# gylien/scale-letkf

Measured on AMD Instinct MI355X. Metric: grid-point LETKF solves/sec, higher is better.
Workload: dtype f64

## Files before the change

### scale-letkf_amd/csrc/letkf_search.hip

```cpp

#include <hip/hip_runtime.h>
#include <limits.h>
#include <stdint.h>
#include <stdio.h>

#include "../../include/letkf_amd.h"
#include "letkf_device.h"
#include "letkf_divby_dev.h"
#include "letkf_lane_dev.h"
#include "letkf_search_dev.h"

namespace letkf {

namespace {

using namespace search_dev;

__device__ __forceinline__ unsigned long long key_bits(int criterion, const CalOut& c) {
  if (criterion == 1) return (unsigned long long)__double_as_longlong(c.ndist);
  if (criterion == 2) return 0x7FFFFFFFFFFFFFFFull - (unsigned long long)__double_as_longlong(c.rloc);
  return (unsigned long long)__double_as_longlong(c.rdiag);
}

enum Pass { kCount = 0, kEmitAll = 1, kHist = 2, kEmitSelect = 3 };

}

struct SelState {
  unsigned long long prefix;
  int shift;
  unsigned long long thresh;
  int tie_budget;
  int emitted;
};

template <int PASS>
__device__ __forceinline__ int sweep_group(const SearchArgs& A, const int gs, const int ge, const double ri,
                                           const double rj, const double rlev, const double rz, const long out,
                                           SelState& st, unsigned int* hist) {
  const letkf_search_tables& t = A.t;
  const int lane = threadIdx.x & 63;
  const unsigned long long lt_mask = (lane == 0) ? 0ull : (~0ull >> (64 - lane));
  int cnt = 0;
  for (int m = gs; m < ge; ++m) {
    const int ic = t.group_member[m];
    const double dzi = t.hori_loc[ic] * kDistZeroFac / t.dx;
    const double dzj = t.hori_loc[ic] * kDistZeroFac / t.dy;
    int imin, imax, jmin, jmax;
    ij_obsgrd_ext(t, ic, ri - dzi, rj - dzj, imin, jmin);
    ij_obsgrd_ext(t, ic, ri + dzi, rj + dzj, imax, jmax);
    imin = max(imin, 1);
    jmin = max(jmin, 1);
    imax = min(imax, t.ngrdext_i[ic]);
    jmax = min(jmax, t.ngrdext_j[ic]);
    if (imin > imax || jmin > jmax) continue;
    const long acb = t.ac_off[ic];
    const int ld = t.ngrdext_i[ic] + 1;
    for (int j = jmin; j <= jmax; ++j) {
      const int lo = t.ac_ext[acb + (imin - 1) + (long)ld * (j - 1)];
      const int hi = t.ac_ext[acb + imax + (long)ld * (j - 1)];
      for (int base = lo; base < hi; base += 64) {
        const int row = base + lane;
        CalOut c{0.0, -1.0, -1.0};
        if (row < hi) c = local_cal(t, ic, ri, rj, rlev, rz, row);
        bool acc = c.rloc != 0.0;
        unsigned long long key = 0;
        if (PASS >= kHist && acc) key = key_bits(t.criterion, c);
        if (PASS == kHist) {
          if (acc && (st.shift == 56 || (key >> (st.shift + 8)) == st.prefix))
            atomicAdd(&hist[(unsigned int)(key >> st.shift) & 0xFFu], 1u);
          continue;
        }
        bool tie = false;
        if (PASS == kEmitSelect) {
          tie = acc && key == st.thresh;
          acc = acc && key < st.thresh;
        }
        const unsigned long long mk = __ballot(acc);
        const int pos = __popcll(mk & lt_mask);
        if (PASS != kCount && acc) {
          const long o = out + st.emitted + pos;
          A.obs_idx[o] = row;
          A.rdiag_l[o] = c.rdiag;
          A.rloc_l[o] = c.rloc;
        }
        const int na = __popcll(mk);
        cnt += na;
        if (PASS != kCount) st.emitted += na;
        if (PASS == kEmitSelect) {
          const unsigned long long tk = __ballot(tie);
          const int tpos = __popcll(tk & lt_mask);
          if (tie && tpos < st.tie_budget) {
            const long o = out + st.emitted + tpos;
            A.obs_idx[o] = row;
            A.rdiag_l[o] = c.rdiag;
            A.rloc_l[o] = c.rloc;
          }
          const int nt = min(__popcll(tk), st.tie_budget);
          st.tie_budget -= nt;
          st.emitted += nt;
          cnt += nt;
        }
      }
    }
  }
  return cnt;
}

__device__ __forceinline__ int wave_incl_scan(int v) {
  v += __builtin_amdgcn_update_dpp(0, v, 0x111, 0xF, 0xF, false);
  v += __builtin_amdgcn_update_dpp(0, v, 0x112, 0xF, 0xF, false);
  v += __builtin_amdgcn_update_dpp(0, v, 0x114, 0xF, 0xF, false);
  v += __builtin_amdgcn_update_dpp(0, v, 0x118, 0xF, 0xF, false);
  v += __builtin_amdgcn_update_dpp(0, v, 0x142, 0xA, 0xF, false);
  v += __builtin_amdgcn_update_dpp(0, v, 0x143, 0xC, 0xF, false);
  return v;
}

__device__ __forceinline__ void find_bin(const unsigned int* hist, const int want, int& bsel, int& before) {
  const int lane = threadIdx.x & 63;
  const uint4 h = *reinterpret_cast<const uint4*>(&hist[4 * lane]);
  const int s = (int)(h.x + h.y + h.z + h.w);
  const int incl = wave_incl_scan(s);
  const int excl = incl - s;
  const bool here = excl < want && incl >= want;
  int b = 4 * lane, cum = excl;
  if (cum + (int)h.x < want) {
    cum += (int)h.x;
    ++b;
    if (cum + (int)h.y < want) {
      cum += (int)h.y;
      ++b;
      if (cum + (int)h.z < want) {
        cum += (int)h.z;
        ++b;
      }
    }
  }
  const unsigned long long mk = __ballot(here);
  if (mk == 0ull) {
    bsel = 255;
    before = __builtin_amdgcn_readlane(incl, 63) - __builtin_amdgcn_readfirstlane((int)hist[255]);
    return;
  }
  const int src = __ffsll((long long)mk) - 1;
  bsel = __builtin_amdgcn_readlane(b, src);
  before = __builtin_amdgcn_readlane(cum, src);
}

constexpr int kCacheCap = 512;

__device__ __forceinline__ int cache_group(const SearchArgs& A, const int gs, const int ge, const double ri,
                                           const double rj, const double rlev, const double rz, double* cache) {
  const letkf_search_tables& t = A.t;
  const int lane = threadIdx.x & 63;
  const unsigned long long lt_mask = (lane == 0) ? 0ull : (~0ull >> (64 - lane));
  int cnt = 0;
  for (int m = gs; m < ge; ++m) {
    const int ic = t.group_member[m];
    const double dzi = t.hori_loc[ic] * kDistZeroFac / t.dx;
    const double dzj = t.hori_loc[ic] * kDistZeroFac / t.dy;
    int imin, imax, jmin, jmax;
    ij_obsgrd_ext(t, ic, ri - dzi, rj - dzj, imin, jmin);
    ij_obsgrd_ext(t, ic, ri + dzi, rj + dzj, imax, jmax);
    imin = max(imin, 1);
    jmin = max(jmin, 1);
    imax = min(imax, t.ngrdext_i[ic]);
    jmax = min(jmax, t.ngrdext_j[ic]);
    if (imin > imax || jmin > jmax) continue;
    const long acb = t.ac_off[ic];
    const int ld = t.ngrdext_i[ic] + 1;
    for (int j = jmin; j <= jmax; ++j) {
      const int lo = t.ac_ext[acb + (imin - 1) + (long)ld * (j - 1)];
      const int hi = t.ac_ext[acb + imax + (long)ld * (j - 1)];
      for (int base = lo; base < hi; base += 64) {
        const int row = base + lane;
        CalOut c{0.0, -1.0, -1.0};
        if (row < hi) c = local_cal(t, ic, ri, rj, rlev, rz, row);
        const bool acc = c.rloc != 0.0;
        const unsigned long long mk = __ballot(acc);
        const int na = __popcll(mk);
        if (cnt + na > kCacheCap) return -1;
        if (acc) {
          const int e = cnt + __popcll(mk & lt_mask);
          *reinterpret_cast<double2*>(&cache[4 * e]) =
              double2{__longlong_as_double((long long)key_bits(t.criterion, c)), __longlong_as_double((long long)row)};
          *reinterpret_cast<double2*>(&cache[4 * e + 2]) = double2{c.rdiag, c.rloc};
        }
        cnt += na;
      }
    }
  }
  return cnt;
}

__device__ __forceinline__ int select_from_cache(const SearchArgs& A, const int nc, const int nmax, const long out,
                                                 const double* cache, unsigned int* hist) {
  const int lane = threadIdx.x & 63;
  const unsigned long long lt_mask = (lane == 0) ? 0ull : (~0ull >> (64 - lane));
  __builtin_amdgcn_fence(__ATOMIC_RELEASE, "wavefront");
  __builtin_amdgcn_wave_barrier();
  __builtin_amdgcn_fence(__ATOMIC_ACQUIRE, "wavefront");
  unsigned long long thresh = ~0ull;
  int tie_budget = 0;
  if (nc > nmax) {
    unsigned long long prefix = 0ull;
    int want = nmax;
    for (int round = 0; round < 8; ++round) {
      for (int b = lane; b < 256; b += 64) hist[b] = 0;
      __builtin_amdgcn_fence(__ATOMIC_RELEASE, "wavefront");
      __builtin_amdgcn_wave_barrier();
      const int shift = 56 - 8 * round;
      for (int e = lane; e < nc; e += 64) {
        const unsigned long long key = (unsigned long long)__double_as_longlong(cache[4 * e]);
        if (round == 0 || (key >> (shift + 8)) == prefix) atomicAdd(&hist[(unsigned int)(key >> shift) & 0xFFu], 1u);
      }
      __builtin_amdgcn_fence(__ATOMIC_ACQ_REL, "wavefront");
      __builtin_amdgcn_wave_barrier();
      int cum = 0, bsel = 255;
      find_bin(hist, want, bsel, cum);
      want -= cum;
      prefix = (round == 0) ? (unsigned long long)bsel : ((prefix << 8) | (unsigned long long)bsel);
    }
    thresh = prefix;
    tie_budget = want;
  }
  int emitted = 0;
  for (int e0 = 0; e0 < nc; e0 += 64) {
    const int e = e0 + lane;
    bool acc = false, tie = false;
    double2 a2{0.0, 0.0}, b2{0.0, 0.0};
    if (e < nc) {
      a2 = *reinterpret_cast<const double2*>(&cache[4 * e]);
      b2 = *reinterpret_cast<const double2*>(&cache[4 * e + 2]);
      const unsigned long long key = (unsigned long long)__double_as_longlong(a2.x);
      acc = nc <= nmax || key < thresh;
      tie = nc > nmax && key == thresh;
    }
    const unsigned long long mk = __ballot(acc);
    if (acc) {
      const long o = out + emitted + __popcll(mk & lt_mask);
      A.obs_idx[o] = (int)__double_as_longlong(a2.y);
      A.rdiag_l[o] = b2.x;
      A.rloc_l[o] = b2.y;
    }
    emitted += __popcll(mk);
    const unsigned long long tk = __ballot(tie);
    const int tpos = __popcll(tk & lt_mask);
    if (tie && tpos < tie_budget) {
      const long o = out + emitted + tpos;
      A.obs_idx[o] = (int)__double_as_longlong(a2.y);
      A.rdiag_l[o] = b2.x;
      A.rloc_l[o] = b2.y;
    }
    const int nt = min(__popcll(tk), tie_budget);
    tie_budget -= nt;
    emitted += nt;
  }
  return emitted;
}

__global__ void __launch_bounds__(256) letkf_search_kernel(const SearchArgs A) {
  __shared__ unsigned int hist_all[4][256];
  extern __shared__ __attribute__((aligned(16))) double cache_all[];
  const letkf_search_tables& t = A.t;
  const int lane = threadIdx.x & 63;
  const int wv = __builtin_amdgcn_readfirstlane(threadIdx.x >> 6);
  unsigned int* hist = hist_all[wv];
  double* cache = cache_all + (size_t)wv * 4 * kCacheCap;

  for (long pt = (long)blockIdx.x * 4 + wv; pt < A.npts; pt += (long)gridDim.x * 4) {
    const double ri = A.ri[pt], rj = A.rj[pt], rlev = A.rlev[pt], rz = A.rz[pt];
    long out = A.fill ? A.obs_off[pt] : 0;
    int total = 0;

    for (int ig = 0; ig < t.ngroup; ++ig) {
      const int gs = t.group_start[ig], ge = t.group_start[ig + 1];
      const int nmax = t.max_nobs[t.group_member[gs]];
      SelState st{0ull, 56, 0ull, 0, 0};
      int ngrp = 0;
      if (nmax <= 0) {
        ngrp = A.fill ? sweep_group<kEmitAll>(A, gs, ge, ri, rj, rlev, rz, out, st, hist)
                      : sweep_group<kCount>(A, gs, ge, ri, rj, rlev, rz, out, st, hist);
      } else if (A.fill && (ngrp = cache_group(A, gs, ge, ri, rj, rlev, rz, cache)) >= 0) {
        ngrp = select_from_cache(A, ngrp, nmax, out, cache, hist);
        __builtin_amdgcn_fence(__ATOMIC_RELEASE, "wavefront");
        __builtin_amdgcn_wave_barrier();
      } else {
        const int cnt = sweep_group<kCount>(A, gs, ge, ri, rj, rlev, rz, out, st, hist);
        if (cnt <= nmax) {
          ngrp = cnt;
          if (A.fill) sweep_group<kEmitAll>(A, gs, ge, ri, rj, rlev, rz, out, st, hist);
        } else if (!A.fill) {
          ngrp = nmax;
        } else {
          int want = nmax;
          for (int round = 0; round < 8; ++round) {
            for (int b = lane; b < 256; b += 64) hist[b] = 0;
            __builtin_amdgcn_fence(__ATOMIC_RELEASE, "wavefront");
            __builtin_amdgcn_wave_barrier();
            st.shift = 56 - 8 * round;
            sweep_group<kHist>(A, gs, ge, ri, rj, rlev, rz, out, st, hist);
            __builtin_amdgcn_fence(__ATOMIC_ACQ_REL, "wavefront");
            __builtin_amdgcn_wave_barrier();
            int cum = 0, bsel = 255;
            find_bin(hist, want, bsel, cum);
            want -= cum;
            st.prefix = (round == 0) ? (unsigned long long)bsel : ((st.prefix << 8) | (unsigned long long)bsel);
          }
          st.thresh = st.prefix;
          st.tie_budget = want;
          st.emitted = 0;
          ngrp = sweep_group<kEmitSelect>(A, gs, ge, ri, rj, rlev, rz, out, st, hist);
        }
      }
      total += ngrp;
      if (A.fill) out += ngrp;
    }
    if (!A.fill && lane == 0) A.counts[pt] = total;
  }
}

constexpr int kSurv = 512;

struct ColArgs {
  letkf_search_tables t;
  long nij1;
  int nlev;
  const double* rig;
  const double* rjg;
  const double* rlev;
  const double* rz;
  int fill;
  int* counts;
  const long* obs_off;
  int* obs_idx;
  double* rdiag_l;
  double* rloc_l;
  int* nobs_ctype;
};

template <bool FILL>
__global__ void __launch_bounds__(256) letkf_search_columns_kernel(const ColArgs A) {
#pragma clang fp contract(off)
  extern __shared__ __attribute__((aligned(16))) double smem_col[];
  const letkf_search_tables& t = A.t;
  const int lane = threadIdx.x & 63;
  const int wv = __builtin_amdgcn_readfirstlane(threadIdx.x >> 6);
  const int nlev = A.nlev;
  const int cstride = 4 * kSurv + 2 * ((nlev + 1) & ~1);
  double* sb = smem_col + (size_t)wv * cstride;
  int* cntl = reinterpret_cast<int*>(sb + 4 * kSurv);
  int* cprev = cntl + 2 * ((nlev + 1) & ~1);
  const unsigned long long lt_mask = (lane == 0) ? 0ull : (~0ull >> (64 - lane));

  for (long col = (long)blockIdx.x * 4 + wv; col < A.nij1; col += (long)gridDim.x * 4) {
    const double ri = A.rig[col], rj = A.rjg[col];
    for (int l = lane; l < nlev; l += 64) cntl[l] = 0;
    __builtin_amdgcn_fence(__ATOMIC_RELEASE, "wavefront");
    __builtin_amdgcn_wave_barrier();
    __builtin_amdgcn_fence(__ATOMIC_ACQUIRE, "wavefront");

    for (int m = 0; m < t.group_start[t.ngroup]; ++m) {
      const int ic = t.group_member[m];
      const double varloc = t.varloc[ic];
      if (varloc < kTiny) continue;
      const int vm = t.vmode[ic];
      const bool wsafe = varloc > 1e-290;
      const double vloc = t.vert_loc[ic], hloc = t.hori_loc[ic];
      const double dzi = hloc * kDistZeroFac / t.dx, dzj = hloc * kDistZeroFac / t.dy;
      int imin, imax, jmin, jmax;
      ij_obsgrd_ext(t, ic, ri - dzi, rj - dzj, imin, jmin);
      ij_obsgrd_ext(t, ic, ri + dzi, rj + dzj, imax, jmax);
      imin = max(imin, 1);
      jmin = max(jmin, 1);
      imax = min(imax, t.ngrdext_i[ic]);
      jmax = min(jmax, t.ngrdext_j[ic]);
      if (imin > imax || jmin > jmax) continue;
      const long acb = t.ac_off[ic];
      const int ld = t.ngrdext_i[ic] + 1;
      int ns = 0;
      if (A.nobs_ctype)
        for (int l = lane; l < nlev; l += 64) cprev[l] = cntl[l];

      auto vertical = [&]() {
        __builtin_amdgcn_fence(__ATOMIC_RELEASE, "wavefront");
        __builtin_amdgcn_wave_barrier();
        __builtin_amdgcn_fence(__ATOMIC_ACQUIRE, "wavefront");
        for (int lev = 0; lev < nlev; ++lev) {
          const long p = col + A.nij1 * (long)lev;
          double vref = 0.0;
          if (vloc != 0.0) {
            if (vm == 1) vref = A.rz[p];
            else vref = log(A.rlev[p]);
          }
          const double vconst = (vm == 3 && vloc != 0.0) ? fabs(log(t.rain_base) - vref) / vloc : 0.0;
          int emitted = cntl[lev];
          const long out = FILL ? A.obs_off[p] : 0;
          for (int s0 = 0; s0 < ns; s0 += 64) {
            const int si = s0 + lane;
            bool acc = false;
            double rloc = 0.0, rdiag = 0.0;
            int row = 0;
            if (si < ns) {
              const double2 a2 = *reinterpret_cast<const double2*>(&sb[4 * si]);
              const double2 b2 = *reinterpret_cast<const double2*>(&sb[4 * si + 2]);
              row = (int)__double_as_longlong(a2.x);
              const double nd_h = a2.y;
              double nd_v;
              if (vloc == 0.0) nd_v = 0.0;
              else if (vm == 3) nd_v = vconst;
              else nd_v = fabs(b2.x - vref) / vloc;
              if (!(nd_v > kDistZeroFac)) {
                const double nd = nd_h * nd_h + nd_v * nd_v;
                if (!(nd > kDistZeroFacSq)) {
                  if (FILL || !wsafe) {
                    rloc = varloc * exp(-0.5 * nd);
                    rdiag = b2.y * b2.y / rloc;
                    acc = rloc != 0.0;
                  } else {
                    acc = true;
                  }
                }
              }
            }
            const unsigned long long mk = __ballot(acc);
            if (FILL && acc) {
              const long o = out + emitted + __popcll(mk & lt_mask);
              A.obs_idx[o] = row;
              A.rdiag_l[o] = rdiag;
              A.rloc_l[o] = rloc;
            }
            emitted += __popcll(mk);
          }
          if (lane == 0) cntl[lev] = emitted;
        }
        __builtin_amdgcn_fence(__ATOMIC_RELEASE, "wavefront");
        __builtin_amdgcn_wave_barrier();
        __builtin_amdgcn_fence(__ATOMIC_ACQUIRE, "wavefront");
        ns = 0;
      };

      for (int j = jmin; j <= jmax; ++j) {
        const int lo = t.ac_ext[acb + (imin - 1) + (long)ld * (j - 1)];
        const int hi = t.ac_ext[acb + imax + (long)ld * (j - 1)];
        for (int base = lo; base < hi; base += 64) {
          const int row = base + lane;
          bool ok = false;
          double nd_h = 0.0, vobs = 0.0, err = 0.0;
          if (row < hi) {
            const double rdx = (ri - t.ob_ri[row]) * t.dx;
            const double rdy = (rj - t.ob_rj[row]) * t.dy;
            nd_h = sqrt(rdx * rdx + rdy * rdy) / hloc;
            ok = !(nd_h > kDistZeroFac);
            if (ok) {
              if (vloc != 0.0) {
                if (vm == 1) vobs = t.ob_lev[row];
                else if (vm == 2) vobs = log(t.ob_dat[row]);
                else if (vm != 3) vobs = log(t.ob_lev[row]);
              }
              err = t.ob_err[row];
            }
          }
          const unsigned long long mk = __ballot(ok);
          if (ok) {
            const int si = ns + __popcll(mk & lt_mask);
            *reinterpret_cast<double2*>(&sb[4 * si]) = double2{__longlong_as_double((long)row), nd_h};
            *reinterpret_cast<double2*>(&sb[4 * si + 2]) = double2{vobs, err};
          }
          ns += __popcll(mk);
          if (ns > kSurv - 64) vertical();
        }
      }
      if (ns > 0) vertical();
      if (A.nobs_ctype)
        for (int l = lane; l < nlev; l += 64)
          A.nobs_ctype[(col + A.nij1 * (long)l) * t.nctype + ic] = cntl[l] - cprev[l];
    }
    if (!FILL)
      for (int l = lane; l < nlev; l += 64) A.counts[col + A.nij1 * (long)l] = cntl[l];
    __builtin_amdgcn_fence(__ATOMIC_RELEASE, "wavefront");
    __builtin_amdgcn_wave_barrier();
    __builtin_amdgcn_fence(__ATOMIC_ACQUIRE, "wavefront");
  }
}


constexpr int kSurvL = 576;
constexpr int kKeyS = kSurvL / 64;
constexpr unsigned long long kNoKey = ~0ull;

struct VertOut {
  double nd, rloc, rdiag;
  bool acc;
};
__device__ __forceinline__ VertOut vertical_cal(const int vm, const double vloc, const double varloc, const double vconst,
                                                const double vref, const double nd_h, const double vobs, const double err) {
#pragma clang fp contract(off)
  VertOut o{0.0, 0.0, 0.0, false};
  double nd_v;
  if (vloc == 0.0) nd_v = 0.0;
  else if (vm == 3) nd_v = vconst;
  else nd_v = fabs(vobs - vref) / vloc;
  if (nd_v > kDistZeroFac) return o;
  const double nd = nd_h * nd_h + nd_v * nd_v;
  if (nd > kDistZeroFacSq) return o;
  o.nd = nd;
  o.rloc = varloc * exp(-0.5 * nd);
  o.rdiag = err * err / o.rloc;
  o.acc = o.rloc != 0.0;
  return o;
}

__device__ __forceinline__ VertOut vertical_nd(const int vm, const double vloc, const double varloc, const double vconst,
                                               const double vref, const double nd_h, const double vobs, const double err) {
#pragma clang fp contract(off)
  if (varloc < 1e-290) return vertical_cal(vm, vloc, varloc, vconst, vref, nd_h, vobs, err);
  VertOut o{0.0, 0.0, 0.0, false};
  double nd_v;
  if (vloc == 0.0) nd_v = 0.0;
  else if (vm == 3) nd_v = vconst;
  else nd_v = fabs(vobs - vref) / vloc;
  if (nd_v > kDistZeroFac) return o;
  const double nd = nd_h * nd_h + nd_v * nd_v;
  if (nd > kDistZeroFacSq) return o;
  o.nd = nd;
  o.acc = true;
  return o;
}

__device__ __forceinline__ unsigned int wave_min_u32(unsigned int v) {
  v = min(v, (unsigned int)__builtin_amdgcn_update_dpp(-1, (int)v, 0x111, 0xF, 0xF, false));
  v = min(v, (unsigned int)__builtin_amdgcn_update_dpp(-1, (int)v, 0x112, 0xF, 0xF, false));
  v = min(v, (unsigned int)__builtin_amdgcn_update_dpp(-1, (int)v, 0x114, 0xF, 0xF, false));
  v = min(v, (unsigned int)__builtin_amdgcn_update_dpp(-1, (int)v, 0x118, 0xF, 0xF, false));
  v = min(v, (unsigned int)__builtin_amdgcn_update_dpp(-1, (int)v, 0x142, 0xA, 0xF, false));
  v = min(v, (unsigned int)__builtin_amdgcn_update_dpp(-1, (int)v, 0x143, 0xC, 0xF, false));
  return (unsigned int)__builtin_amdgcn_readlane((int)v, 63);
}
__device__ __forceinline__ unsigned int wave_max_u32(unsigned int v) {
  v = max(v, (unsigned int)__builtin_amdgcn_update_dpp(0, (int)v, 0x111, 0xF, 0xF, false));
  v = max(v, (unsigned int)__builtin_amdgcn_update_dpp(0, (int)v, 0x112, 0xF, 0xF, false));
  v = max(v, (unsigned int)__builtin_amdgcn_update_dpp(0, (int)v, 0x114, 0xF, 0xF, false));
  v = max(v, (unsigned int)__builtin_amdgcn_update_dpp(0, (int)v, 0x118, 0xF, 0xF, false));
  v = max(v, (unsigned int)__builtin_amdgcn_update_dpp(0, (int)v, 0x142, 0xA, 0xF, false));
  v = max(v, (unsigned int)__builtin_amdgcn_update_dpp(0, (int)v, 0x143, 0xC, 0xF, false));
  return (unsigned int)__builtin_amdgcn_readlane((int)v, 63);
}
using lane_dev::mbcnt;
using lane_dev::uniform;
using lane_dev::wave_lds_sync;

template <int KS>
__device__ __forceinline__ void hist_thresh(const unsigned long long (&key_in)[KS], const int ns, const int nreal, int want,
                                            unsigned int* hist, unsigned long long& thresh, int& tie_budget,
                                            const double lin_scale = 0.0) {
  const int lane = threadIdx.x & 63;
  const unsigned long long lt_mask = (lane == 0) ? 0ull : (~0ull >> (64 - lane));
  unsigned long long key[KS];
#pragma unroll
  for (int u = 0; u < KS; ++u) key[u] = key_in[u];
  int inclass = nreal;
  if (lin_scale > 0.0 && inclass > 64) {
    *reinterpret_cast<uint4*>(&hist[4 * lane]) = uint4{0u, 0u, 0u, 0u};
    wave_lds_sync();
    int dig[KS];
#pragma unroll
    for (int u = 0; u < KS; ++u) {
      dig[u] = min((int)(__longlong_as_double((long long)key[u]) * lin_scale), 255);
      if (u * 64 < ns && key[u] != kNoKey) atomicAdd(&hist[dig[u]], 1u);
    }
    wave_lds_sync();
    int bsel = 0, before = 0;
    find_bin(hist, want, bsel, before);
    const int cb = (int)hist[bsel];
    wave_lds_sync();
    want -= before;
    inclass = __builtin_amdgcn_readfirstlane(cb);
#pragma unroll
    for (int u = 0; u < KS; ++u)
      if (dig[u] != bsel) key[u] = kNoKey;
  }
  unsigned long long lo = 0ull, hi = 1ull << 63;
  if (inclass > 64) {
    unsigned int mn = ~0u, mx = 0u;
#pragma unroll
    for (int u = 0; u < KS; ++u) {
      const unsigned int h = (unsigned int)(key[u] >> 32);
      mn = min(mn, h);
      mx = max(mx, key[u] != kNoKey ? h : 0u);
    }
    lo = (unsigned long long)wave_min_u32(mn) << 32;
    hi = ((unsigned long long)wave_max_u32(mx) + 1ull) << 32;
  }
  while (inclass > 64) {
    const unsigned long long span1 = hi - lo - 1ull;
    if (span1 == 0ull) {
      thresh = lo;
      tie_budget = want;
      return;
    }
    const int w = 64 - __clzll((long long)span1);
    const int sh = w > 8 ? w - 8 : 0;
    *reinterpret_cast<uint4*>(&hist[4 * lane]) = uint4{0u, 0u, 0u, 0u};
    wave_lds_sync();
#pragma unroll
    for (int u = 0; u < KS; ++u)
      if (u * 64 < ns && key[u] >= lo && key[u] < hi) atomicAdd(&hist[(unsigned int)((key[u] - lo) >> sh)], 1u);
    wave_lds_sync();
    int bsel = 0, before = 0;
    find_bin(hist, want, bsel, before);
    const int cb = (int)hist[bsel];
    wave_lds_sync();
    want -= before;
    inclass = __builtin_amdgcn_readfirstlane(cb);
    lo += (unsigned long long)bsel << sh;
    const unsigned long long top = lo + (1ull << sh);
    hi = top < hi ? top : hi;
  }
  unsigned long long* cbuf = reinterpret_cast<unsigned long long*>(hist);
  int base = 0;
#pragma unroll
  for (int u = 0; u < KS; ++u)
    if (u * 64 < ns) {
      const bool in = key[u] >= lo && key[u] < hi;
      const unsigned long long m = __ballot(in);
      if (in) cbuf[base + __popcll(m & lt_mask)] = key[u];
      base += __popcll(m);
    }
  wave_lds_sync();
  const unsigned long long mine = lane < inclass ? cbuf[lane] : kNoKey;
  int r_lt = 0, r_le = 0;
  for (int j = 0; j < inclass; ++j) {
    const unsigned long long kj = cbuf[j];
    r_lt += kj < mine;
    r_le += kj <= mine;
  }
  const unsigned long long hit = __ballot(lane < inclass && r_lt < want && r_le >= want);
  const int src = __ffsll((long long)hit) - 1;
  thresh = ((unsigned long long)(unsigned int)__builtin_amdgcn_readlane((int)(mine >> 32), src) << 32) |
           (unsigned int)__builtin_amdgcn_readlane((int)mine, src);
  tie_budget = want - __builtin_amdgcn_readlane(r_lt, src);
  wave_lds_sync();
}

#ifdef LETKF_WAVE_PROF
__device__ unsigned long long g_lim_prof[8];
#define LP_T() __builtin_readcyclecounter()
#define LP_ADD(i, v) lpa[i] += (unsigned long long)(v)
#define LP_DECL() unsigned long long lpa[8] = {0, 0, 0, 0, 0, 0, 0, 0}
#define LP_FLUSH() do { if (lane == 0) for (int i = 0; i < 8; ++i) atomicAdd(&g_lim_prof[i], lpa[i]); } while (0)
#else
#define LP_DECL() do {} while (0)
#define LP_FLUSH() do {} while (0)
#define LP_T() 0ull
#define LP_ADD(i, v) do {} while (0)
#endif
struct ColLimArgs {
  ColArgs c;
  double* cutd_ctype;
};

__global__ void __launch_bounds__(256, 2) letkf_search_columns_limited_kernel(const ColLimArgs L) {
#pragma clang fp contract(off)
  extern __shared__ __attribute__((aligned(16))) double smem_lim[];
  __shared__ __attribute__((aligned(16))) unsigned int hist_all[4][kSurvL / 2];
  const ColArgs& A = L.c;
  const letkf_search_tables& t = A.t;
  const int lane = threadIdx.x & 63;
  const int wv = __builtin_amdgcn_readfirstlane(threadIdx.x >> 6);
  const int nlev = A.nlev;
  const int nl2 = (nlev + 1) & ~1;
  const int cstride = 4 * kSurvL + nl2;
  double* sb = smem_lim + (size_t)wv * cstride;
  int* cntl = reinterpret_cast<int*>(sb + 4 * kSurvL);
  unsigned int* hist = hist_all[wv];
  const unsigned long long lt_mask = (lane == 0) ? 0ull : (~0ull >> (64 - lane));
  SearchArgs PA;
  PA.t = t;
  PA.fill = A.fill;
  PA.obs_idx = A.obs_idx;
  PA.rdiag_l = A.rdiag_l;
  PA.rloc_l = A.rloc_l;

  LP_DECL();
  for (long col = (long)blockIdx.x * 4 + wv; col < A.nij1; col += (long)gridDim.x * 4) {
    const double ri = A.rig[col], rj = A.rjg[col];
    for (int l = lane; l < nlev; l += 64) cntl[l] = 0;
    if (A.nobs_ctype || L.cutd_ctype)
      for (int e = lane; e < nlev * t.nctype; e += 64) {
        const int l = e / t.nctype, ic = e - l * t.nctype;
        const long p = col + A.nij1 * (long)l;
        if (A.nobs_ctype) A.nobs_ctype[p * t.nctype + ic] = 0;
        if (L.cutd_ctype) L.cutd_ctype[p * t.nctype + ic] = 0.0;
      }
    __builtin_amdgcn_fence(__ATOMIC_RELEASE, "wavefront");
    __builtin_amdgcn_wave_barrier();
    __builtin_amdgcn_fence(__ATOMIC_ACQUIRE, "wavefront");

    for (int ig = 0; ig < t.ngroup; ++ig) {
      const int gs = t.group_start[ig], ge = t.group_start[ig + 1];
      const int icm = t.group_member[gs];
      const int nmax = t.max_nobs[icm];
      [[maybe_unused]] const unsigned long long lp0 = LP_T();
      int ns = 0;
      bool overflow = ge - gs > 4;
      int mbeg[4] = {INT_MAX, INT_MAX, INT_MAX, INT_MAX}, mend[4] = {0, 0, 0, 0};
      for (int m = gs; m < ge && !overflow; ++m) {
        const int ic = t.group_member[m];
        ns = (ns + 63) & ~63;
        const int ns0 = ns;
        const bool skip = t.varloc[ic] < kTiny;
        const int vm = t.vmode[ic];
        const double vloc = t.vert_loc[ic], hloc = t.hori_loc[ic];
        const double dzi = hloc * kDistZeroFac / t.dx, dzj = hloc * kDistZeroFac / t.dy;
        int imin, imax, jmin, jmax;
        ij_obsgrd_ext(t, ic, ri - dzi, rj - dzj, imin, jmin);
        ij_obsgrd_ext(t, ic, ri + dzi, rj + dzj, imax, jmax);
        imin = max(imin, 1);
        jmin = max(jmin, 1);
        imax = min(imax, t.ngrdext_i[ic]);
        jmax = min(jmax, t.ngrdext_j[ic]);
        if (skip || imin > imax) jmax = jmin - 1;
        const long acb = t.ac_off[ic];
        const int ld = t.ngrdext_i[ic] + 1;
        for (int j = jmin; j <= jmax && !overflow; ++j) {
          const int lo = t.ac_ext[acb + (imin - 1) + (long)ld * (j - 1)];
          const int hi = t.ac_ext[acb + imax + (long)ld * (j - 1)];
          for (int base = lo; base < hi; base += 64) {
            const int row = base + lane;
            bool ok = false;
            double nd_h = 0.0, vobs = 0.0, err = 0.0;
            if (row < hi) {
              const double rdx = (ri - t.ob_ri[row]) * t.dx;
              const double rdy = (rj - t.ob_rj[row]) * t.dy;
              nd_h = sqrt(rdx * rdx + rdy * rdy) / hloc;
              ok = !(nd_h > kDistZeroFac);
              if (ok) {
                if (vloc != 0.0) {
                  if (vm == 1) vobs = t.ob_lev[row];
                  else if (vm == 2) vobs = log(t.ob_dat[row]);
                  else if (vm != 3) vobs = log(t.ob_lev[row]);
                }
                err = t.ob_err[row];
              }
            }
            const unsigned long long mk = __ballot(ok);
            const int na = __popcll(mk);
            if (ns + na > kSurvL) {
              overflow = true;
              break;
            }
            if (ok) {
              const int si = ns + __popcll(mk & lt_mask);
              *reinterpret_cast<double2*>(&sb[4 * si]) = double2{nd_h, vobs};
              *reinterpret_cast<double2*>(&sb[4 * si + 2]) = double2{__longlong_as_double((long)row), err};
            }
            ns += na;
          }
        }
#pragma unroll
        for (int q = 0; q < 4; ++q)
          if (m - gs == q) {
            mbeg[q] = ns0;
            mend[q] = ns;
          }
      }
      wave_lds_sync();
      ns = uniform(ns);
      overflow = uniform((int)overflow) != 0;
      LP_ADD(0, LP_T() - lp0);
      LP_ADD(6, ns);
      const double cut_default = (t.criterion == 1) ? t.hori_loc[icm] * kDistZeroFac : 0.0;
      int vm_m[4], ic_m[4];
      double vloc_m[4], varloc_m[4];
      bool fast = nmax > 0 && t.criterion == 1 && ge - gs <= 2 && !overflow;
#pragma unroll
      for (int mo = 0; mo < 4; ++mo) {
        const int ic = t.group_member[min(gs + mo, ge - 1)];
        ic_m[mo] = uniform(ic);
        vm_m[mo] = uniform(t.vmode[ic]);
        vloc_m[mo] = uniform(t.vert_loc[ic]);
        varloc_m[mo] = uniform(t.varloc[ic]);
        if (varloc_m[mo] < 1e-290) fast = false;
        if (vloc_m[mo] != 0.0 && !divby::in_range(vloc_m[mo])) fast = false;
      }
      const bool count_only = !A.fill && !L.cutd_ctype && nmax > 0;
      const int mbeg1 = uniform(mbeg[1]);
      double yv_m[2];
#pragma unroll
      for (int q = 0; q < 2; ++q) yv_m[q] = uniform(divby::reciprocal(vloc_m[q]));
      double ndh2_r[kKeyS], vobs_r[kKeyS];
      if (fast) {
#pragma unroll
        for (int u = 0; u < kKeyS; ++u) {
          ndh2_r[u] = __longlong_as_double(0x7FF0000000000000ll);
          vobs_r[u] = 0.0;
          if (u * 64 >= ns) continue;
          const int si = u * 64 + lane;
          const int me = u * 64 >= mbeg1 ? mend[1] : mend[0];
          if (si < me) {
            const double2 a2 = *reinterpret_cast<const double2*>(&sb[4 * si]);
            ndh2_r[u] = a2.x * a2.x;
            vobs_r[u] = a2.y;
          }
        }
      }

      for (int lev = 0; lev < nlev; ++lev) {
        const long p = col + A.nij1 * (long)lev;
        const long out = (A.fill ? A.obs_off[p] : 0) + cntl[lev];
        int nsel = 0;
        double cutd = cut_default;
        int cm[4] = {0, 0, 0, 0};
        if (overflow) {
          const double rlev = A.rlev[p], rz = A.rz[p];
          SelState st{0ull, 56, 0ull, 0, 0};
          if (nmax <= 0) {
            nsel = A.fill ? sweep_group<kEmitAll>(PA, gs, ge, ri, rj, rlev, rz, out, st, hist)
                          : sweep_group<kCount>(PA, gs, ge, ri, rj, rlev, rz, out, st, hist);
          } else {
            const int cnt = sweep_group<kCount>(PA, gs, ge, ri, rj, rlev, rz, out, st, hist);
            if (cnt <= nmax) {
              nsel = cnt;
              if (A.fill) sweep_group<kEmitAll>(PA, gs, ge, ri, rj, rlev, rz, out, st, hist);
            } else {
              nsel = nmax;
              if (A.fill || L.cutd_ctype) {
                int want = nmax;
                for (int round = 0; round < 8; ++round) {
                  for (int b = lane; b < 256; b += 64) hist[b] = 0;
                  __builtin_amdgcn_fence(__ATOMIC_RELEASE, "wavefront");
                  __builtin_amdgcn_wave_barrier();
                  st.shift = 56 - 8 * round;
                  sweep_group<kHist>(PA, gs, ge, ri, rj, rlev, rz, out, st, hist);
                  __builtin_amdgcn_fence(__ATOMIC_ACQ_REL, "wavefront");
                  __builtin_amdgcn_wave_barrier();
                  int cum = 0, bsel = 255;
                  find_bin(hist, want, bsel, cum);
                  want -= cum;
                  st.prefix = (round == 0) ? (unsigned long long)bsel : ((st.prefix << 8) | (unsigned long long)bsel);
                }
                st.thresh = st.prefix;
                st.tie_budget = want;
                st.emitted = 0;
                if (A.fill) sweep_group<kEmitSelect>(PA, gs, ge, ri, rj, rlev, rz, out, st, hist);
                const double kv = __longlong_as_double((long long)(t.criterion == 2 ? 0x7FFFFFFFFFFFFFFFull - st.thresh : st.thresh));
                cutd = (t.criterion == 1) ? t.hori_loc[icm] * sqrt(kv) : kv;
              }
            }
          }
        } else {
          const double vz = uniform(A.rz[p]), vlnp = uniform(log(A.rlev[p]));
          const double lnrain = uniform(log(t.rain_base));
// ... 469 lines not shown
            }
            wave_lds_sync();
          }
        } else {
          const bool count_only = !A.fill && !A.cutd_ctype;
          int nB = 0, tot = 0, pos = 0, rp = 0;
          unsigned long long tau = kNoKey;
          while (pos < n_g) {
            while (rp + 1 < kRings && ro[rp + 1] <= pos) ++rp;
            if (count_only && tot >= nmax) break;
            if (nB == nmax) {
              if constexpr (!GEN) {
                const double lb = (double)rp * (1.0 / kRingScale) * (1.0 - 1e-12);
                if ((unsigned long long)__double_as_longlong(lb) >= tau) break;
              } else if (rp > 0) {
                const double edge = (double)rp * (1.0 / kRingScale) + A.kref[ig];
                const unsigned long long lbk =
                    t.criterion == 2 ? 0x7FFFFFFFFFFFFFFFull - (unsigned long long)__double_as_longlong(exp(-0.5 * edge) * (1.0 + 1e-9))
                                     : (unsigned long long)__double_as_longlong(exp(0.5 * edge) * (1.0 - 1e-9));
                if (lbk >= tau) break;
              }
            }
            const int nbs = (nB + 63) >> 6;
            unsigned long long keyr[kRingSlots];
            long rwr[kRingSlots];
            double errr[kRingSlots];
            int nreal = 0, nnew = 0;
            double2 ta[kRingSlots], tb[kRingSlots];
#pragma unroll
            for (int u = 0; u < kRingSlots; ++u) {
              const int e = min(pos + (u - nbs) * 64 + lane, n_g - 1);
              const long ea = e0 + (u >= nbs ? e : 0);
              ta[u] = *reinterpret_cast<const double2*>(&A.sv[4 * ea]);
              tb[u] = *reinterpret_cast<const double2*>(&A.sv[4 * ea + 2]);
            }
#pragma unroll
            for (int u = 0; u < kRingSlots; ++u) {
              keyr[u] = kNoKey;
              rwr[u] = 0;
              errr[u] = 0.0;
              if (u < nbs) {
                const int j = u * 64 + lane;
                if (j < nB) {
                  keyr[u] = bkey[j];
                  rwr[u] = brw[j];
                  errr[u] = berr[j];
                }
              } else {
                const int e = pos + (u - nbs) * 64 + lane;
                double nd;
                if (e < n_g && entry_key(ta[u], tb[u], nd)) {
                  rwr[u] = __double_as_longlong(ta[u].x);
                  if constexpr (!GEN) {
                    keyr[u] = (unsigned long long)__double_as_longlong(nd);
                    errr[u] = tb[u].y;
                  } else {
                    const double rloc = s_varloc[(int)(rwr[u] >> 32)] * exp(-0.5 * nd);
                    if (t.criterion == 2) {
                      keyr[u] = 0x7FFFFFFFFFFFFFFFull - (unsigned long long)__double_as_longlong(rloc);
                      errr[u] = tb[u].y;
                    } else {
                      keyr[u] = (unsigned long long)__double_as_longlong(tb[u].y * tb[u].y / rloc);
                      errr[u] = rloc;
                    }
                  }
                }
              }
              const int c = __popcll(__ballot(keyr[u] != kNoKey));
              nreal += c;
              if (u >= nbs) nnew += c;
            }
            tot += nnew;
            pos += (kRingSlots - nbs) * 64;
            if (count_only) continue;
            wave_lds_sync();
            unsigned long long thresh = kNoKey;
            int tie_budget = 0;
            if (nreal > nmax) hist_thresh<kRingSlots>(keyr, kRingSlots * 64, nreal, nmax, hist, thresh, tie_budget, GEN ? 0.0 : 256.0 / 13.5);
            tie_budget = uniform(tie_budget);
            const bool ties = thresh != kNoKey;
            int nl = 0;
#pragma unroll
            for (int u = 0; u < kRingSlots; ++u) {
              const bool take = keyr[u] < thresh, tie = ties && keyr[u] == thresh;
              const unsigned long long mk = __ballot(take), tk = __ballot(tie);
              const int nm = __popcll(mk), tpos = mbcnt(tk);
              if (take || (tie && tpos < tie_budget)) {
                const int j = nl + (take ? mbcnt(mk) : nm + tpos);
                bkey[j] = keyr[u];
                brw[j] = rwr[u];
                berr[j] = errr[u];
              }
              const int nt = min((int)__popcll(tk), tie_budget);
              tie_budget -= nt;
              nl += nm + nt;
            }
            nB = nl;
            if (nreal >= nmax) {
              if (nreal > nmax) tau = thresh;
              else {
                unsigned int hi = 0u;
#pragma unroll
                for (int u = 0; u < kRingSlots; ++u)
                  if (keyr[u] != kNoKey) hi = max(hi, (unsigned int)(keyr[u] >> 32));
                tau = ((unsigned long long)wave_max_u32(hi) + 1ull) << 32;
              }
            }
            wave_lds_sync();
          }
          nsel = count_only ? min(tot, nmax) : nB;
          if (!count_only && nB == nmax) {
            unsigned long long kmx = 0ull;
            for (int j = lane; j < nB; j += 64) kmx = bkey[j] > kmx ? bkey[j] : kmx;
            const unsigned int hmx = wave_max_u32((unsigned int)(kmx >> 32));
            unsigned int lmx = ((unsigned int)(kmx >> 32) == hmx) ? (unsigned int)kmx : 0u;
            lmx = wave_max_u32(lmx);
            const double kv = __longlong_as_double((long long)(((unsigned long long)hmx << 32) | lmx));
            if constexpr (!GEN) cutd = (t.criterion == 1) ? t.hori_loc[icm] * sqrt(kv) : s_varloc[icm] * exp(-0.5 * kv);
            else
              cutd = t.criterion == 2 ? __longlong_as_double((long long)(0x7FFFFFFFFFFFFFFFull - (((unsigned long long)hmx << 32) | lmx))) : kv;
          }
          if (A.fill) {
            for (int j = lane; j < nB; j += 64) {
              const long rw = brw[j];
              const int ic = (int)(rw >> 32);
              double rloc, rdiag;
              if constexpr (!GEN) {
                const double nd = __longlong_as_double((long long)bkey[j]);
                rloc = s_varloc[ic] * exp(-0.5 * nd);
                rdiag = berr[j] * berr[j] / rloc;
              } else if (t.criterion == 2) {
                rloc = __longlong_as_double((long long)(0x7FFFFFFFFFFFFFFFull - bkey[j]));
                rdiag = berr[j] * berr[j] / rloc;
              } else {
                rloc = berr[j];
                rdiag = __longlong_as_double((long long)bkey[j]);
              }
              const long o = out0 + emitted + j;
              A.obs_idx[o] = (int)(rw & 0xffffffffL);
              A.rdiag_l[o] = rdiag;
              A.rloc_l[o] = rloc;
            }
          }
          if (lane == 0) {
            if (A.nobs_ctype) A.nobs_ctype[p * t.nctype + icm] = nsel;
            if (A.cutd_ctype) A.cutd_ctype[p * t.nctype + icm] = cutd;
          }
          wave_lds_sync();
        }
        emitted += nsel;
      }
      if (!A.fill && lane == 0) A.counts[p] = emitted;
    }
  }
}

__global__ void __launch_bounds__(256) letkf_ctype_min_err_kernel(const letkf_search_tables t, double* out) {
  __shared__ double red[256];
  const int ic = blockIdx.x;
  const long acb = t.ac_off[ic];
  const long nac = (long)(t.ngrdext_i[ic] + 1) * t.ngrdext_j[ic];
  const int lo = t.ac_ext[acb], hi = t.ac_ext[acb + nac - 1];
  double m = 1e300;
  for (int r = lo + threadIdx.x; r < hi; r += 256) m = fmin(m, t.ob_err[r]);
  red[threadIdx.x] = m;
  __syncthreads();
  for (int s_ = 128; s_ > 0; s_ >>= 1) {
    if ((int)threadIdx.x < s_) red[threadIdx.x] = fmin(red[threadIdx.x], red[threadIdx.x + s_]);
    __syncthreads();
  }
  if (threadIdx.x == 0) out[ic] = red[0];
}
hipError_t launch_ctype_min_err(const letkf_search_tables& t, double* out, hipStream_t st) {
  hipLaunchKernelGGL(letkf_ctype_min_err_kernel, dim3(t.nctype), dim3(256), 0, st, t, out);
  return hipGetLastError();
}

hipError_t launch_ring_survivors(const letkf_search_tables& t, long col0, long ncol, const double* rig, const double* rjg, int fill,
                                 int* counts, const long* goff, double* sv, int* roff, const double* kref, int num_cu, hipStream_t st) {
  if (ncol <= 0) return hipSuccess;
  RingBuildArgs a{t, col0, ncol, rig, rjg, counts, goff, sv, roff, kref != nullptr ? 1 : 0, kref};
  const long nwg = (ncol + 3) / 4;
  const long g = (long)num_cu * 8;
  const int grid = (int)(nwg < g ? nwg : g);
  if (fill) hipLaunchKernelGGL(letkf_ring_survivors_kernel<true>, dim3(grid), dim3(256), 0, st, a);
  else hipLaunchKernelGGL(letkf_ring_survivors_kernel<false>, dim3(grid), dim3(256), 0, st, a);
  return hipGetLastError();
}

hipError_t launch_search_rings(const letkf_search_tables& t, long col0, long ncol, long nij1, int nlev, const double* rlev,
                               const double* rz, int fill, int* counts, const long* obs_off, int* obs_idx, double* rdiag_l,
                               double* rloc_l, int* nobs_ctype, double* cutd_ctype, const long* goff, const double* sv,
                               const int* roff, const double* kref, int num_cu, hipStream_t st) {
  if (ncol <= 0) return hipSuccess;
  RingSearchArgs a{t, col0, ncol, nij1, nlev, rlev, rz, fill, counts, obs_off, obs_idx, rdiag_l, rloc_l, nobs_ctype, cutd_ctype,
                   goff, sv, roff, kref};
  const long nwg = (ncol + 3) / 4;
  const long g = (long)num_cu * 4;
  const int grid = (int)(nwg < g ? nwg : g);
  if (kref) hipLaunchKernelGGL(letkf_search_rings_kernel<true>, dim3(grid), dim3(256), 0, st, a);
  else hipLaunchKernelGGL(letkf_search_rings_kernel<false>, dim3(grid), dim3(256), 0, st, a);
  return hipGetLastError();
}

int search_rings_max_nobs() { return kRingSel; }
int search_rings_count() { return kRings; }
int search_rings_lds_survivors() { return kSurvL; }

struct SurvArgs {
  letkf_search_tables t;
  long col0, ncol;
  const double *rig, *rjg;
  int* counts;
  const long* sv_off;
  double* sv;
};

template <bool FILL>
__global__ void __launch_bounds__(256) letkf_survivors_kernel(const SurvArgs A) {
#pragma clang fp contract(off)
  const letkf_search_tables& t = A.t;
  const int lane = threadIdx.x & 63;
  const int wv = __builtin_amdgcn_readfirstlane(threadIdx.x >> 6);
  const unsigned long long lt_mask = (lane == 0) ? 0ull : (~0ull >> (64 - lane));
  for (long cb = (long)blockIdx.x * 4 + wv; cb < A.ncol; cb += (long)gridDim.x * 4) {
    const long col = A.col0 + cb;
    const double ri = A.rig[col], rj = A.rjg[col];
    long ns = 0;
    const long out = FILL ? A.sv_off[cb] : 0;
    for (int m = 0; m < t.group_start[t.ngroup]; ++m) {
      const int ic = t.group_member[m];
      if (t.varloc[ic] < kTiny) continue;
      const int vm = t.vmode[ic];
      const double vloc = t.vert_loc[ic], hloc = t.hori_loc[ic];
      const double dzi = hloc * kDistZeroFac / t.dx, dzj = hloc * kDistZeroFac / t.dy;
      int imin, imax, jmin, jmax;
      ij_obsgrd_ext(t, ic, ri - dzi, rj - dzj, imin, jmin);
      ij_obsgrd_ext(t, ic, ri + dzi, rj + dzj, imax, jmax);
      imin = max(imin, 1);
      jmin = max(jmin, 1);
      imax = min(imax, t.ngrdext_i[ic]);
      jmax = min(jmax, t.ngrdext_j[ic]);
      if (imin > imax || jmin > jmax) continue;
      const long acb = t.ac_off[ic];
      const int ld = t.ngrdext_i[ic] + 1;
      for (int j = jmin; j <= jmax; ++j) {
        const int lo = t.ac_ext[acb + (imin - 1) + (long)ld * (j - 1)];
        const int hi = t.ac_ext[acb + imax + (long)ld * (j - 1)];
        for (int base = lo; base < hi; base += 64) {
          const int row = base + lane;
          bool ok = false;
          double nd_h = 0.0;
          if (row < hi) {
            const double rdx = (ri - t.ob_ri[row]) * t.dx;
            const double rdy = (rj - t.ob_rj[row]) * t.dy;
            nd_h = sqrt(rdx * rdx + rdy * rdy) / hloc;
            ok = !(nd_h > kDistZeroFac);
          }
          const unsigned long long mk = __ballot(ok);
          if (FILL && ok) {
            double vobs = 0.0;
            if (vloc != 0.0) {
              if (vm == 1) vobs = t.ob_lev[row];
              else if (vm == 2) vobs = log(t.ob_dat[row]);
              else if (vm != 3) vobs = log(t.ob_lev[row]);
            }
            const long o = 4 * (out + ns + __popcll(mk & lt_mask));
            const long rw = (long)row | ((long)ic << 32);
            *reinterpret_cast<double2*>(&A.sv[o]) = double2{__longlong_as_double(rw), nd_h};
            *reinterpret_cast<double2*>(&A.sv[o + 2]) = double2{vobs, t.ob_err[row]};
          }
          ns += __popcll(mk);
        }
      }
      const long npad = (64 - (ns & 63)) & 63;
      if (FILL && lane < npad) {
        const long o = 4 * (out + ns + lane);
        *reinterpret_cast<double2*>(&A.sv[o]) = double2{__longlong_as_double((long)ic << 32), 1e30};
        *reinterpret_cast<double2*>(&A.sv[o + 2]) = double2{0.0, 1.0};
      }
      ns += npad;
    }
    if (!FILL && lane == 0) A.counts[cb] = (int)ns;
  }
}

hipError_t launch_survivors(const letkf_search_tables& t, long col0, long ncol, const double* rig, const double* rjg, int fill,
                            int* counts, const long* sv_off, double* sv, int num_cu, hipStream_t st) {
  if (ncol <= 0) return hipSuccess;
  SurvArgs a{t, col0, ncol, rig, rjg, counts, sv_off, sv};
  const long nwg = (ncol + 3) / 4;
  const long g = (long)num_cu * 8;
  const int grid = (int)(nwg < g ? nwg : g);
  if (fill) hipLaunchKernelGGL(letkf_survivors_kernel<true>, dim3(grid), dim3(256), 0, st, a);
  else hipLaunchKernelGGL(letkf_survivors_kernel<false>, dim3(grid), dim3(256), 0, st, a);
  return hipGetLastError();
}

hipError_t launch_search_columns(const letkf_search_tables& t, long nij1, int nlev, const double* rig,
                                 const double* rjg, const double* rlev, const double* rz, int fill, int* counts,
                                 const long* obs_off, int* obs_idx, double* rdiag_l, double* rloc_l, int* nobs_ctype,
                                 int num_cu, hipStream_t st) {
  ColArgs a{t, nij1, nlev, rig, rjg, rlev, rz, fill, counts, obs_off, obs_idx, rdiag_l, rloc_l, nobs_ctype};
  const size_t lds = (size_t)4 * (4 * kSurv + 2 * ((nlev + 1) & ~1)) * sizeof(double);
  auto kern = fill ? &letkf_search_columns_kernel<true> : &letkf_search_columns_kernel<false>;
  if (hipError_t e = lds_opt_in(kern, lds)) return e;
  const long nwg = (nij1 + 3) / 4;
  const long g = (long)num_cu * 8;
  const int grid = (int)(nwg < g ? (nwg > 0 ? nwg : 1) : g);
  hipLaunchKernelGGL(kern, dim3(grid), dim3(256), lds, st, a);
  return hipGetLastError();
}

hipError_t launch_search(const SearchArgs& a, int num_cu, hipStream_t st) {
  const long nwg = (a.npts + 3) / 4;
  const long g = (long)num_cu * 8;
  const int grid = (int)(nwg < g ? (nwg > 0 ? nwg : 1) : g);
  const size_t lds = a.limited ? (size_t)4 * 4 * kCacheCap * sizeof(double) : 0;
  if (hipError_t e = lds_opt_in(&letkf_search_kernel, lds)) return e;
  hipLaunchKernelGGL(letkf_search_kernel, dim3(grid), dim3(256), lds, st, a);
  return hipGetLastError();
}

}
```

Measured before the change: 9.790 million.

## Restructure column search vertical pass with SoA survivors, compaction queue, per-level counting

Reworks the column-search kernel's vertical pass. Survivor storage moves from interleaved 4-double records to split arrays, with a smaller fill-mode buffer. Fill mode now compacts cutoff-passing candidates into an LDS ring queue before the exp/divide and global stores. Count mode can give each lane its own level and loop over survivors, and vertical distances use a precomputed reciprocal division specialised per vertical mode. The grid cap rises from 8 to 64 workgroups per CU. These aim to cut divergent exp work, LDS traffic and scattered stores, at the cost of more code paths and extra queue synchronisation.

```diff
diff --git a/scale-letkf_amd/csrc/letkf_search.hip b/scale-letkf_amd/csrc/letkf_search.hip
--- a/scale-letkf_amd/csrc/letkf_search.hip
+++ b/scale-letkf_amd/csrc/letkf_search.hip
@@ -3,6 +3,8 @@
 #include <limits.h>
 #include <stdint.h>
 #include <stdio.h>
+
+#include <type_traits>
 
 #include "../../include/letkf_amd.h"
 #include "letkf_device.h"
@@ -321,7 +323,22 @@
   }
 }
 
+using lane_dev::mbcnt;
+using lane_dev::readlane_d;
+using lane_dev::uniform;
+using lane_dev::wave_lds_sync;
+
+#ifndef LETKF_COL_SURV_FILL
+#define LETKF_COL_SURV_FILL 384
+#endif
 constexpr int kSurv = 512;
+constexpr int kSurvFill = LETKF_COL_SURV_FILL;
+constexpr int kColQueue = 128;
+static_assert(kSurv % 64 == 0 && kSurvFill % 64 == 0 && kSurvFill <= kSurv, "survivor buffers hold whole chunks");
+
+__host__ __device__ constexpr size_t col_wave_bytes(const bool fill, const int nlev) {
+  return (fill ? (size_t)kSurvFill * 28 + kColQueue * 12 : (size_t)kSurv * 16) + 8 * (size_t)((nlev + 1) & ~1);
+}
 
 struct ColArgs {
   letkf_search_tables t;
@@ -340,34 +357,55 @@
   int* nobs_ctype;
 };
 
+template <int MODE>
+__device__ __forceinline__ bool col_cutoff(const double2 hv, const double vref, const double ndv_c, const double vloc,
+                                           const double yv, double& nd) {
+#pragma clang fp contract(off)
+  double nd_v;
+  if (MODE == 0) {
+    nd_v = ndv_c;
+  } else {
+    const double a = fabs(hv.y - vref);
+    nd_v = MODE == 1 ? divby::quotient(a, vloc, yv) : a / vloc;
+  }
+  nd = hv.x * hv.x + nd_v * nd_v;
+  return !(nd_v > kDistZeroFac) && !(nd > kDistZeroFacSq);
+}
+
 template <bool FILL>
 __global__ void __launch_bounds__(256) letkf_search_columns_kernel(const ColArgs A) {
 #pragma clang fp contract(off)
   extern __shared__ __attribute__((aligned(16))) double smem_col[];
+  constexpr int kS = FILL ? kSurvFill : kSurv;
   const letkf_search_tables& t = A.t;
   const int lane = threadIdx.x & 63;
   const int wv = __builtin_amdgcn_readfirstlane(threadIdx.x >> 6);
   const int nlev = A.nlev;
-  const int cstride = 4 * kSurv + 2 * ((nlev + 1) & ~1);
-  double* sb = smem_col + (size_t)wv * cstride;
-  int* cntl = reinterpret_cast<int*>(sb + 4 * kSurv);
-  int* cprev = cntl + 2 * ((nlev + 1) & ~1);
-  const unsigned long long lt_mask = (lane == 0) ? 0ull : (~0ull >> (64 - lane));
+  const int nl2 = (nlev + 1) & ~1;
+  char* wb = reinterpret_cast<char*>(smem_col) + (size_t)wv * col_wave_bytes(FILL, nlev);
+  double2* s_hv = reinterpret_cast<double2*>(wb);
+  double* s_err = reinterpret_cast<double*>(s_hv + kS);
+  double* q_nd = s_err + kS;
+  int* s_row = reinterpret_cast<int*>(q_nd + kColQueue);
+  int* q_si = s_row + kS;
+  int* cntl = FILL ? q_si + kColQueue : reinterpret_cast<int*>(s_hv + kS);
+  int* cprev = cntl + nl2;
+  const bool by_level = !FILL && 2 * nlev >= 64 * ((nlev + 63) / 64);
 
   for (long col = (long)blockIdx.x * 4 + wv; col < A.nij1; col += (long)gridDim.x * 4) {
     const double ri = A.rig[col], rj = A.rjg[col];
     for (int l = lane; l < nlev; l += 64) cntl[l] = 0;
-    __builtin_amdgcn_fence(__ATOMIC_RELEASE, "wavefront");
-    __builtin_amdgcn_wave_barrier();
-    __builtin_amdgcn_fence(__ATOMIC_ACQUIRE, "wavefront");
+    wave_lds_sync();
 
     for (int m = 0; m < t.group_start[t.ngroup]; ++m) {
       const int ic = t.group_member[m];
-      const double varloc = t.varloc[ic];
+      const double varloc = uniform(t.varloc[ic]);
       if (varloc < kTiny) continue;
-      const int vm = t.vmode[ic];
+      const int vm = uniform(t.vmode[ic]);
       const bool wsafe = varloc > 1e-290;
-      const double vloc = t.vert_loc[ic], hloc = t.hori_loc[ic];
+      const double vloc = uniform(t.vert_loc[ic]), hloc = t.hori_loc[ic];
+      const bool fdiv = divby::in_range(vloc);
+      const double yv = uniform(divby::reciprocal(fdiv ? vloc : 1.0));
       const double dzi = hloc * kDistZeroFac / t.dx, dzj = hloc * kDistZeroFac / t.dy;
       int imin, imax, jmin, jmax;
       ij_obsgrd_ext(t, ic, ri - dzi, rj - dzj, imin, jmin);
@@ -383,68 +421,117 @@
       if (A.nobs_ctype)
         for (int l = lane; l < nlev; l += 64) cprev[l] = cntl[l];
 
-      auto vertical = [&]() {
-        __builtin_amdgcn_fence(__ATOMIC_RELEASE, "wavefront");
-        __builtin_amdgcn_wave_barrier();
-        __builtin_amdgcn_fence(__ATOMIC_ACQUIRE, "wavefront");
-        for (int lev = 0; lev < nlev; ++lev) {
-          const long p = col + A.nij1 * (long)lev;
-          double vref = 0.0;
-          if (vloc != 0.0) {
-            if (vm == 1) vref = A.rz[p];
-            else vref = log(A.rlev[p]);
-          }
-          const double vconst = (vm == 3 && vloc != 0.0) ? fabs(log(t.rain_base) - vref) / vloc : 0.0;
-          int emitted = cntl[lev];
-          const long out = FILL ? A.obs_off[p] : 0;
-          for (int s0 = 0; s0 < ns; s0 += 64) {
-            const int si = s0 + lane;
-            bool acc = false;
-            double rloc = 0.0, rdiag = 0.0;
-            int row = 0;
-            if (si < ns) {
-              const double2 a2 = *reinterpret_cast<const double2*>(&sb[4 * si]);
-              const double2 b2 = *reinterpret_cast<const double2*>(&sb[4 * si + 2]);
-              row = (int)__double_as_longlong(a2.x);
-              const double nd_h = a2.y;
-              double nd_v;
-              if (vloc == 0.0) nd_v = 0.0;
-              else if (vm == 3) nd_v = vconst;
-              else nd_v = fabs(b2.x - vref) / vloc;
-              if (!(nd_v > kDistZeroFac)) {
-                const double nd = nd_h * nd_h + nd_v * nd_v;
-                if (!(nd > kDistZeroFacSq)) {
-                  if (FILL || !wsafe) {
+      auto level_ref = [&](const long p, double& vref, double& ndv_c) {
+        vref = 0.0;
+        if (vloc != 0.0) {
+          if (vm == 1) vref = A.rz[p];
+          else vref = log(A.rlev[p]);
+        }
+        ndv_c = (vm == 3 && vloc != 0.0) ? fabs(log(t.rain_base) - vref) / vloc : 0.0;
+      };
+
+      auto vertical_mode = [&](auto mode_c) {
+        constexpr int MODE = decltype(mode_c)::value;
+        wave_lds_sync();
+        if (!FILL && wsafe && by_level) {
+          for (int l0 = 0; l0 < nlev; l0 += 64) {
+            const int lev = min(l0 + lane, nlev - 1);
+            double vref, ndv_c;
+            level_ref(col + A.nij1 * (long)lev, vref, ndv_c);
+            int c = 0;
+#pragma unroll 4
+            for (int s = 0; s < ns; ++s) {
+              double nd;
+              c += col_cutoff<MODE>(s_hv[s], vref, ndv_c, vloc, yv, nd) ? 1 : 0;
+            }
+            if (l0 + lane < nlev) cntl[l0 + lane] += c;
+          }
+        } else {
+          int head = 0;
+          for (int l0 = 0; l0 < nlev; l0 += 64) {
+            const int ll = min(l0 + lane, nlev - 1);
+            const long pl = col + A.nij1 * (long)ll;
+            double vref_v, ndv_v;
+            level_ref(pl, vref_v, ndv_v);
+            const long out_v = FILL ? A.obs_off[pl] : 0;
+            int cnt_v = cntl[ll];
+            const int nl = min(64, nlev - l0);
+            for (int k = 0; k < nl; ++k) {
+              const double vref = readlane_d(vref_v, k), ndv_c = readlane_d(ndv_v, k);
+              int emitted = __builtin_amdgcn_readlane(cnt_v, k);
+              if (FILL) {
+                const long out = ((long)__builtin_amdgcn_readlane((int)(out_v >> 32), k) << 32) |
+                                 (unsigned int)__builtin_amdgcn_readlane((int)out_v, k);
+                int nq = 0;
+                auto drain = [&](const int n) {
+                  wave_lds_sync();
+                  bool acc = false;
+                  double rloc = 0.0, rdiag = 0.0;
+                  int row = 0;
+                  if (lane < n) {
+                    const int q = (head + lane) & (kColQueue - 1);
+                    const int si = q_si[q];
+                    const double nd = q_nd[q], err = s_err[si];
+                    row = s_row[si];
                     rloc = varloc * exp(-0.5 * nd);
-                    rdiag = b2.y * b2.y / rloc;
+                    rdiag = err * err / rloc;
                     acc = rloc != 0.0;
-                  } else {
-                    acc = true;
                   }
+                  const unsigned long long mk = __ballot(acc);
+                  if (acc) {
+                    const long o = out + emitted + mbcnt(mk);
+                    A.obs_idx[o] = row;
+                    A.rdiag_l[o] = rdiag;
+                    A.rloc_l[o] = rloc;
+                  }
+                  emitted += __popcll(mk);
+                  head = (head + n) & (kColQueue - 1);
+                  nq -= n;
+                };
+                for (int s0 = 0; s0 < ns; s0 += 64) {
+                  const int si = s0 + lane;
+                  double nd = 0.0;
+                  bool cand = false;
+                  if (si < ns) cand = col_cutoff<MODE>(s_hv[si], vref, ndv_c, vloc, yv, nd);
+                  const unsigned long long mk = __ballot(cand);
+                  if (cand) {
+                    const int q = (head + nq + mbcnt(mk)) & (kColQueue - 1);
+                    q_nd[q] = nd;
+                    q_si[q] = si;
+                  }
+                  nq += __popcll(mk);
+                  if (nq >= 64) drain(64);
                 }
-              }
-            }
-            const unsigned long long mk = __ballot(acc);
-            if (FILL && acc) {
-              const long o = out + emitted + __popcll(mk & lt_mask);
-              A.obs_idx[o] = row;
-              A.rdiag_l[o] = rdiag;
-              A.rloc_l[o] = rloc;
-            }
-            emitted += __popcll(mk);
-          }
-          if (lane == 0) cntl[lev] = emitted;
+                if (nq > 0) drain(nq);
+              } else {
+                for (int s0 = 0; s0 < ns; s0 += 64) {
+                  const int si = s0 + lane;
+                  double nd = 0.0;
+                  bool acc = false;
+                  if (si < ns) acc = col_cutoff<MODE>(s_hv[si], vref, ndv_c, vloc, yv, nd);
+                  if (!wsafe && acc) acc = varloc * exp(-0.5 * nd) != 0.0;
+                  emitted += __popcll(__ballot(acc));
+                }
+              }
+              if (lane == k) cnt_v = emitted;
+            }
+            if (l0 + lane < nlev) cntl[l0 + lane] = cnt_v;
+          }
         }
-        __builtin_amdgcn_fence(__ATOMIC_RELEASE, "wavefront");
-        __builtin_amdgcn_wave_barrier();
-        __builtin_amdgcn_fence(__ATOMIC_ACQUIRE, "wavefront");
+        wave_lds_sync();
         ns = 0;
       };
-
-      for (int j = jmin; j <= jmax; ++j) {
-        const int lo = t.ac_ext[acb + (imin - 1) + (long)ld * (j - 1)];
-        const int hi = t.ac_ext[acb + imax + (long)ld * (j - 1)];
-        for (int base = lo; base < hi; base += 64) {
+      auto vertical = [&]() {
+        if (vloc == 0.0 || vm == 3) vertical_mode(std::integral_constant<int, 0>{});
+        else if (fdiv) vertical_mode(std::integral_constant<int, 1>{});
+        else vertical_mode(std::integral_constant<int, 2>{});
+      };
+
+      for (int j = jmin; j <= jmax + 1; ++j) {
+        const bool last = j > jmax;
+        const int lo = last ? 0 : t.ac_ext[acb + (imin - 1) + (long)ld * (j - 1)];
+        const int hi = last ? 0 : t.ac_ext[acb + imax + (long)ld * (j - 1)];
+        for (int base = lo; base < hi || (last && base == 0 && ns > 0); base += 64) {
           const int row = base + lane;
           bool ok = false;
           double nd_h = 0.0, vobs = 0.0, err = 0.0;
@@ -459,29 +546,29 @@
                 else if (vm == 2) vobs = log(t.ob_dat[row]);
                 else if (vm != 3) vobs = log(t.ob_lev[row]);
               }
-              err = t.ob_err[row];
+              if (FILL) err = t.ob_err[row];
             }
           }
           const unsigned long long mk = __ballot(ok);
           if (ok) {
-            const int si = ns + __popcll(mk & lt_mask);
-            *reinterpret_cast<double2*>(&sb[4 * si]) = double2{__longlong_as_double((long)row), nd_h};
-            *reinterpret_cast<double2*>(&sb[4 * si + 2]) = double2{vobs, err};
+            const int si = ns + mbcnt(mk);
+            s_hv[si] = double2{nd_h, vobs};
+            if (FILL) {
+              s_err[si] = err;
+              s_row[si] = row;
+            }
           }
           ns += __popcll(mk);
-          if (ns > kSurv - 64) vertical();
+          if (ns > kS - 64 || last) vertical();
         }
       }
-      if (ns > 0) vertical();
       if (A.nobs_ctype)
         for (int l = lane; l < nlev; l += 64)
           A.nobs_ctype[(col + A.nij1 * (long)l) * t.nctype + ic] = cntl[l] - cprev[l];
     }
     if (!FILL)
       for (int l = lane; l < nlev; l += 64) A.counts[col + A.nij1 * (long)l] = cntl[l];
-    __builtin_amdgcn_fence(__ATOMIC_RELEASE, "wavefront");
-    __builtin_amdgcn_wave_barrier();
-    __builtin_amdgcn_fence(__ATOMIC_ACQUIRE, "wavefront");
+    wave_lds_sync();
   }
 }
 
@@ -547,9 +634,6 @@
   v = max(v, (unsigned int)__builtin_amdgcn_update_dpp(0, (int)v, 0x143, 0xC, 0xF, false));
   return (unsigned int)__builtin_amdgcn_readlane((int)v, 63);
 }
-using lane_dev::mbcnt;
-using lane_dev::uniform;
-using lane_dev::wave_lds_sync;
 
 template <int KS>
 __device__ __forceinline__ void hist_thresh(const unsigned long long (&key_in)[KS], const int ns, const int nreal, int want,
@@ -1625,11 +1709,11 @@
                                  const long* obs_off, int* obs_idx, double* rdiag_l, double* rloc_l, int* nobs_ctype,
                                  int num_cu, hipStream_t st) {
   ColArgs a{t, nij1, nlev, rig, rjg, rlev, rz, fill, counts, obs_off, obs_idx, rdiag_l, rloc_l, nobs_ctype};
-  const size_t lds = (size_t)4 * (4 * kSurv + 2 * ((nlev + 1) & ~1)) * sizeof(double);
+  const size_t lds = 4 * col_wave_bytes(fill != 0, nlev);
   auto kern = fill ? &letkf_search_columns_kernel<true> : &letkf_search_columns_kernel<false>;
   if (hipError_t e = lds_opt_in(kern, lds)) return e;
   const long nwg = (nij1 + 3) / 4;
-  const long g = (long)num_cu * 8;
+  const long g = (long)num_cu * 64;
   const int grid = (int)(nwg < g ? (nwg > 0 ? nwg : 1) : g);
   hipLaunchKernelGGL(kern, dim3(grid), dim3(256), lds, st, a);
   return hipGetLastError();
```

Measured after the change: 9.951 million (median of 6 runs). 1.6% higher.
